# naver/deep-image-retrieval

Hardware: AMD Instinct MI355X
Metric: images/sec descriptor extraction (resnet101-GeM, 1024x1024) (higher is better)
Workload: dtype fp16p

## Files before the change

### deep-image-retrieval_amd/csrc/conv_igemm.hip

```cpp
#include "dir_common.h"
#include "conv_igemm.h"

#include <stdlib.h>
#include <string.h>
#include <algorithm>

namespace dir {

static constexpr uint32_t kOOB = 0x80000000u;

__device__ __forceinline__ void dma16(__amdgpu_buffer_rsrc_t rsrc, char* lds, uint32_t voff, int soff) {
    __builtin_amdgcn_raw_ptr_buffer_load_lds(rsrc, (DIR_LDS void*)lds, 16, voff, soff, 0, 0);
}

__device__ inline uint32_t fast_div(uint32_t n, uint32_t mul, uint32_t shr) {
    return mul ? (__umulhi(n, mul) >> shr) : n;
}

template <class DT, int BM, int BN, int WGM, int WGN, int NST, int BK, bool CIN16, bool SPLITK>
__global__ void __launch_bounds__(64 * WGM * WGN) conv_igemm_kernel(const ConvArgs a) {
    static_assert(NST >= 2 && NST <= 8, "ring depth");
    static_assert((BK == 64 || BK == 32) && (!CIN16 || BK == 64), "K-step");
    constexpr int RB = BK * 2;
    constexpr int CPR = BK / 8;
// ... 552 lines not shown

int conv_pick_dual_variant(const ConvArgs& a, bool any_size) {
    const bool ok = a.x2 && a.R == 1 && a.S == 1 && a.stride == 1 && a.pad == 0 && a.H == a.OH && a.W == a.OW &&
                    a.Cin % 64 == 0 && a.Cin2 % 64 == 0 && a.res == nullptr && a.ksplit <= 1;
    if (!ok) return -1;
    {
        const int v = find_variant("64x256_wregd1x1");
        if (v >= 0 && !env().no_wregd && conv1x1_wregd_admissible(a) &&
            (any_size || (long)ceil_div(a.M, 64) * (a.Cout / 256) >= 1024))
            return v;
    }
    if (a.Cout % 256 != 0 || (!any_size && (long)ceil_div(a.M, 256) * (a.Cout / 256) < 192)) return -1;
    if (env().lc1x1) {
        const int vl = find_variant("256x256_lc1x1");
        if (vl >= 0 && conv1x1_lc_admissible(a)) return vl;
    }
    const int v = find_variant("256x256_persist1x1_x3");
    if (v < 0 || kVariants[v].launch_dual[0] == nullptr) return -1;
    return v;
}

template <class DT>
__global__ void conv_splitk_finalize_kernel(const float* __restrict__ partial, const float* __restrict__ bias,
                                            const uint16_t* res, uint16_t* y,
                                            long total8, int Cout, long MC, int ksplit, int relu, int* ovf_flag) {
    const long i8 = (long)blockIdx.x * blockDim.x + threadIdx.x;
    if (i8 >= total8) return;
    const long o = i8 * 8;
    const int n = (int)(o % Cout);
    float v[8];
    const f32x4_t b0 = *(const DIR_GLOBAL f32x4_t*)(bias + n), b1 = *(const DIR_GLOBAL f32x4_t*)(bias + n + 4);
#pragma unroll
    for (int e = 0; e < 4; ++e) v[e] = b0[e], v[4 + e] = b1[e];
    for (int z = 0; z < ksplit; ++z) {
        const float* p = partial + (size_t)z * MC + o;
        const f32x4_t p0 = *(const DIR_GLOBAL f32x4_t*)p, p1 = *(const DIR_GLOBAL f32x4_t*)(p + 4);
#pragma unroll
        for (int e = 0; e < 4; ++e) v[e] += p0[e], v[4 + e] += p1[e];
    }
    if (res) {
        const u32x4_t rv = gload16(res + o);
#pragma unroll
        for (int e = 0; e < 4; ++e) {
            float lo, hi;
            DT::unpack(rv[e], lo, hi);
            v[2 * e] += lo;
            v[2 * e + 1] += hi;
        }
    }
    if (relu) {
#pragma unroll
        for (int e = 0; e < 8; ++e) v[e] = fmaxf(v[e], 0.f);
    }
    u32x4_t ov;
#pragma unroll
    for (int e = 0; e < 4; ++e) ov[e] = DT::pack(v[2 * e], v[2 * e + 1]);
    gstore16(y + o, ov);
    Ovf<DT> ovf;
    ovf.see(ov);
    ovf.flush(ovf_flag);
}

size_t conv_splitk_bytes(const ConvArgs& a, int ksplit) {
    return ksplit > 1 ? (size_t)ksplit * a.M * a.Cout * sizeof(float) : 0;
}

int conv_splitk_factor(int v, const ConvArgs& a) {
    if (v < 0 || v >= kNumVariants || kVariants[v].launch_sk[0] == nullptr || a.Cin == 16) return 1;
    const ConvVariant& cv = kVariants[v];
    const long tiles = (long)ceil_div(a.M, cv.BM) * (a.Cout / cv.BN);
    const int T = a.Ktot / cv.BK;
    if (tiles > 160 || T < 8) return 1;
    int s = (int)std::min<long>(std::min<long>(8, 512 / tiles), T / 4);
    while (s > 1 && conv_splitk_bytes(a, s) > kSplitKMaxBytes) --s;
    return s < 2 ? 1 : s;
}

int conv_launch(const ConvArgs& a, int dtype, int variant, hipStream_t stream) {
    if (a.Cout % 64 != 0) return fail(DIR_ERR_INVALID, "conv: Cout must be a multiple of 64");
    const bool cin16 = (a.Cin == 16);
    if (cin16) {
        if (a.R != 4 || a.S != 4 || a.stride != 1)
            return fail(DIR_ERR_INVALID, "conv: Cin == 16 is only the 4x4 s1 space-to-depth stem");
    } else if (a.Cin % 64 != 0) {
        return fail(DIR_ERR_INVALID, "conv: Cin must be a multiple of 64 (or 16 for the stem)");
    }
    if (a.R > 4 || a.S > 4) return fail(DIR_ERR_INVALID, "conv: filter larger than 4x4");
    if ((long)a.B * a.H * a.W * a.Cin >= (1L << 30) || (long)a.M * a.Cout >= (1L << 30) ||
        (long)a.Cout * a.Ktot >= (1L << 30))
        return fail(DIR_ERR_INVALID, "conv: tensor exceeds 2^31 bytes; lower the batch");
    if (((uintptr_t)a.x & 15) || ((uintptr_t)a.w & 15) || ((uintptr_t)a.y & 15) ||
        ((uintptr_t)a.res & 15) || ((uintptr_t)a.bias & 15))
        return fail(DIR_ERR_INVALID, "conv: tensors must be 16-byte aligned");
    if (dtype != DIR_BF16 && dtype != DIR_FP16) return fail(DIR_ERR_INVALID, "conv: bad dtype");
    if (a.x2) {
        if (variant < 0) variant = conv_pick_dual_variant(a);
        if (variant < 0 || variant >= kNumVariants || kVariants[variant].launch_dual[0] == nullptr ||
            a.Cout % kVariants[variant].BN != 0 || (kVariants[variant].kind == 9 && !conv1x1_wregd_admissible(a)) || (kVariants[variant].kind == 10 && !conv1x1_lc_admissible(a)) || a.R != 1 || a.S != 1 || a.stride != 1 || a.res || a.ksplit > 1 ||
            a.Cin2 % 64 != 0 || a.Ktot != a.Cin + a.Cin2 || ((uintptr_t)a.x2 & 15) ||
            (long)a.B * a.H2 * a.W2 * a.Cin2 >= (1L << 30))
            return fail(DIR_ERR_INVALID, "conv: no two-source form for this shape / variant");
        hipError_t e = kVariants[variant].launch_dual[dtype](a, stream);
        if (e != hipSuccess)
            return fail(DIR_ERR_HIP, std::string("conv launch ") + kVariants[variant].name + "/dual: " + hipGetErrorString(e));
        return DIR_OK;
    }
    if (variant < 0) variant = conv_pick_variant(a);
    if (!conv_variant_admissible(variant, a))
        return fail(DIR_ERR_INVALID, "conv: variant not admissible for this shape");
    const ConvVariant& cv = kVariants[variant];
    if (a.ksplit > 1) {
        if (cv.launch_sk[0] == nullptr || cin16)
            return fail(DIR_ERR_INVALID, "conv: this variant has no split-K form");
        if (!a.partial || ((uintptr_t)a.partial & 15))
            return fail(DIR_ERR_INVALID, "conv: split-K needs a 16-byte aligned fp32 scratch buffer");
        if (a.ksplit > a.Ktot / cv.BK) return fail(DIR_ERR_INVALID, "conv: more K slices than K-steps");
    }
    hipError_t e = cv.kind == 1   ? conv_patch3x3_launch(a, dtype, stream)
                   : cv.kind == 5 ? conv_patch3x3s_launch(a, dtype, stream)
                   : cv.kind == 6 ? conv_patch3x3w_launch(a, dtype, stream)
                   : cv.kind == 2 ? conv1x1_persist_launch(a, dtype, stream)
                   : cv.kind == 4 ? conv1x1_persist_launch(a, dtype, stream, true)
                   : cv.kind == 3 ? conv1x1_wreg_launch(a, dtype, stream)
#ifdef DIR_EXPERIMENTS
                   : cv.kind == 7 ? conv1x1_ring_launch(a, dtype, stream)
#endif
                   : cv.kind == 8 ? conv_patch64_lc_launch(a, dtype, stream)
                   : cv.kind == 12 ? conv_patch3x3s2_launch(a, dtype, stream)
                   : cv.kind == 10 ? conv1x1_lc_launch(a, dtype, stream)
                   : cv.kind == 11 ? conv_small_launch(a, dtype, cv.stages, stream)
                   : a.ksplit > 1 ? cv.launch_sk[dtype](a, stream)
                                  : (cin16 ? cv.launch16 : cv.launch)[dtype](a, stream);
    if (e != hipSuccess)
        return fail(DIR_ERR_HIP, std::string("conv launch ") + cv.name + ": " + hipGetErrorString(e));
    if (a.ksplit > 1) {
        const long MC = (long)a.M * a.Cout, total8 = MC / 8;
        const dim3 grid((unsigned)((total8 + 255) / 256));
        if (dtype == DIR_BF16)
            hipLaunchKernelGGL(conv_splitk_finalize_kernel<BF16>, grid, dim3(256), 0, stream, a.partial, a.bias,
                               a.res, a.y, total8, a.Cout, MC, a.ksplit, a.relu, a.ovf);
        else
            hipLaunchKernelGGL(conv_splitk_finalize_kernel<FP16>, grid, dim3(256), 0, stream, a.partial, a.bias,
                               a.res, a.y, total8, a.Cout, MC, a.ksplit, a.relu, a.ovf);
        e = hipGetLastError();
        if (e != hipSuccess) return fail(DIR_ERR_HIP, std::string("conv split-K finalize: ") + hipGetErrorString(e));
    }
    return DIR_OK;
}

template <class DT>
__global__ void conv_naive_kernel(const ConvArgs a) {
    const long idx = (long)blockIdx.x * blockDim.x + threadIdx.x;
    if (idx >= (long)a.M * a.Cout) return;
    const int n = (int)(idx % a.Cout);
    const int m = (int)(idx / a.Cout);
    const int OHW = a.OH * a.OW;
    const int b = m / OHW, rem = m - b * OHW, oh = rem / a.OW, ow = rem - oh * a.OW;
    float acc = 0.f;
    for (int r = 0; r < a.R; ++r) {
        const int ih = oh * a.stride - a.pad + r;
        if ((unsigned)ih >= (unsigned)a.H) continue;
        for (int s = 0; s < a.S; ++s) {
            const int iw = ow * a.stride - a.pad + s;
            if ((unsigned)iw >= (unsigned)a.W) continue;
            const uint16_t* xp = a.x + ((size_t)(b * a.H + ih) * a.W + iw) * a.Cin;
            const uint16_t* wp = a.w + (size_t)n * a.Ktot + (r * a.S + s) * a.Cin;
            for (int c = 0; c < a.Cin; ++c) acc = fmaf(DT::to_f32(xp[c]), DT::to_f32(wp[c]), acc);
// ... 24 lines not shown
```

### deep-image-retrieval_amd/csrc/conv_patchw.hip

```cpp
#include "dir_common.h"
#include "conv_igemm.h"

#ifndef DIR_PATCHW_ABL
#define DIR_PATCHW_ABL 0
#endif

namespace dir {

static constexpr uint32_t kOOBw = 0x80000000u;

__device__ __forceinline__ void dma16w(__amdgpu_buffer_rsrc_t rsrc, char* lds, uint32_t voff, int soff) {
    __builtin_amdgcn_raw_ptr_buffer_load_lds(rsrc, (DIR_LDS void*)lds, 16, voff, soff, 0, 0);
}

template <class DT>
__global__ void __launch_bounds__(512) conv_patch3x3w_kernel(const ConvArgs a) {
    constexpr int TH = 16, TW = 32, PH = TH + 2, PW = TW + 2, PP = PH * PW;
    constexpr int NTH = 512, BN = 128;
    constexpr int NPL = (PP * 4 + NTH - 1) / NTH;
    constexpr int PLANE_BYTES = NPL * NTH * 16;
    constexpr int TN = 4, TMR = 2;
    constexpr int WSTAGE = 3 * BN * 64, NBW = WSTAGE / (NTH * 16);
    constexpr int NBW_X = (DIR_PATCHW_ABL & 16) ? 2 : 0;
    constexpr int NPL_X = (DIR_PATCHW_ABL & 32) ? 7 : 0;
    constexpr int NSTW = 3;
    constexpr int WOFF = 2 * PLANE_BYTES;
    constexpr int EROW = TN * 128 + 16;
    typedef typename DT::frag_t frag_t;
    static_assert(WOFF + NSTW * WSTAGE <= 160 * 1024 && NBW * NTH * 16 == WSTAGE, "LDS map");

    extern __shared__ __attribute__((aligned(16))) char smem[];

    const int tid = threadIdx.x;
    const int lane = tid & 63;
    const int wave = __builtin_amdgcn_readfirstlane(tid >> 6);
    const int lrow = lane & 31, lhi = lane >> 5;

    const int NQ = a.Cin / 32;
    const int NS = NQ * 3;
    const int tiles_n = a.Cout / BN;
    const int tiles_x = (a.OW + TW - 1) / TW;
    const int tiles_y = (a.OH + TH - 1) / TH;
    int wg = xcd_remap(blockIdx.x, gridDim.x);
    const int tile_n = wg % tiles_n;
    wg /= tiles_n;
    const int tx = wg % tiles_x;
    wg /= tiles_x;
    const int ty = wg % tiles_y;
    const int b = wg / tiles_y;
    const int oy0 = ty * TH, ox0 = tx * TW;

    const __amdgpu_buffer_rsrc_t rsrc_x = __builtin_amdgcn_make_buffer_rsrc((void*)a.x, 0, a.x_bytes, 0x00020000);
    const __amdgpu_buffer_rsrc_t rsrc_w = __builtin_amdgcn_make_buffer_rsrc((void*)a.w, 0, a.w_bytes, 0x00020000);

    uint32_t pvoff[NPL];
#pragma unroll
    for (int i = 0; i < NPL; ++i) {
        const int P = i * NTH + tid;
        const int p = P >> 2, pos = P & 3;
        const int py = p / PW, px = p - py * PW;
        const int iy = oy0 - 1 + py, ix = ox0 - 1 + px;
        const bool ok = p < PP && (unsigned)iy < (unsigned)a.H && (unsigned)ix < (unsigned)a.W;
        pvoff[i] = ok ? (uint32_t)((((b * a.H + iy) * a.W + ix) * a.Cin + ((pos ^ ((p >> 2) & 3)) << 3)) * 2) : kOOBw;
    }
    auto issue_plane = [&](int q) {
        if (DIR_PATCHW_ABL & 64) return;
        char* dst = smem + (q & 1) * PLANE_BYTES;
#pragma unroll
        for (int i = 0; i < NPL; ++i) dma16w(rsrc_x, dst + (i * NTH + wave * 64) * 16, pvoff[i], q * 64);
#pragma unroll
        for (int rep = 0; rep < NPL_X; ++rep)
#pragma unroll
            for (int i = 0; i < NPL; ++i) dma16w(rsrc_x, dst + (i * NTH + wave * 64) * 16, pvoff[i], q * 64);
    };
    uint32_t wvoff[NBW];
#pragma unroll
    for (int i = 0; i < NBW; ++i) {
        const int L = i * NTH + tid;
        const int s = L >> 9, n = (L & 511) >> 2, pos = L & 3;
        wvoff[i] = (uint32_t)((((tile_n * BN + n) * 9 + s) * a.Cin + ((pos ^ ((n >> 2) & 3)) << 3)) * 2);
    }
    auto issue_w = [&](int sigma, int slot) {
        if (DIR_PATCHW_ABL & 64) return;
        const int q = sigma / 3, r = sigma - q * 3;
        char* dst = smem + WOFF + slot * WSTAGE;
#pragma unroll
        for (int i = 0; i < NBW; ++i) dma16w(rsrc_w, dst + (i * NTH + wave * 64) * 16, wvoff[i], (r * 3 * a.Cin + q * 32) * 2);
#pragma unroll
        for (int i = 0; i < NBW_X; ++i)
            dma16w(rsrc_w, dst + (i * NTH + wave * 64) * 16, wvoff[i], (((r + 1) % 3) * 3 * a.Cin + q * 32) * 2);
    };

    f32x16_t acc[TN][TMR];
#pragma unroll
    for (int i = 0; i < TN; ++i)
#pragma unroll
        for (int g = 0; g < 4; ++g) {
            const f32x4_t b4 = *(const DIR_GLOBAL f32x4_t*)(a.bias + tile_n * BN + i * 32 + 8 * g + 4 * lhi);
#pragma unroll
            for (int j = 0; j < TMR; ++j)
#pragma unroll
                for (int e = 0; e < 4; ++e) acc[i][j][4 * g + e] = b4[e];
        }

    int woffk[2];
#pragma unroll
    for (int kk = 0; kk < 2; ++kk) woffk[kk] = lrow * 64 + (((2 * kk + lhi) ^ ((lrow >> 2) & 3)) << 4);

    issue_plane(0);
    issue_w(0, 0);
    issue_w(1, 1);
    int q = 0, r = 0;
    int slot_c = 0;
    bool plane_before = false;
    for (int sigma = 0; sigma < NS; ++sigma) {
        if (((DIR_PATCHW_ABL & 4) && sigma == 0) || (DIR_PATCHW_ABL & 64)) {
        } else if (sigma + 1 >= NS) {
            asm volatile("s_waitcnt vmcnt(0)" ::: "memory");
        } else if (plane_before) {
            asm volatile("s_waitcnt vmcnt(%0)" ::"i"(NPL * (1 + NPL_X) + NBW + NBW_X) : "memory");
        } else {
            asm volatile("s_waitcnt vmcnt(%0)" ::"i"(NBW + NBW_X) : "memory");
        }
        ring_barrier();
        plane_before = false;
        if (r == 0 && q + 1 < NQ) {
            issue_plane(q + 1);
            plane_before = true;
        }
        if (sigma + 2 < NS) {
            int slot_n = slot_c + 2;
            if (slot_n >= NSTW) slot_n -= NSTW;
            issue_w(sigma + 2, slot_n);
        }
        const char* plane = smem + (q & 1) * PLANE_BYTES;
        const char* wst = smem + WOFF + slot_c * WSTAGE;
#pragma unroll
        for (int s = 0; s < ((DIR_PATCHW_ABL & 128) ? 0 : 3); ++s) {
            frag_t xf[TMR][2], wf[2][TN];
#pragma unroll
            for (int j = 0; j < TMR; ++j) {
                const int p = (wave * TMR + j + r) * PW + s + lrow;
                const int swz = (p >> 2) & 3;
#pragma unroll
                for (int kk = 0; kk < 2; ++kk) xf[j][kk] = *(const frag_t*)(plane + p * 64 + (((2 * kk + lhi) ^ swz) << 4));
            }
#pragma unroll
            for (int kk = 0; kk < 2; ++kk)
#pragma unroll
                for (int i = 0; i < TN; ++i) wf[kk][i] = *(const frag_t*)(wst + s * (BN * 64) + i * 2048 + woffk[kk]);
#pragma unroll
            for (int kk = 0; kk < 2; ++kk)
#pragma unroll
                for (int i = 0; i < TN; ++i)
#pragma unroll
                    for (int j = 0; j < TMR; ++j) {
                        if ((DIR_PATCHW_ABL & 8) && !(s == 0 || (s == 1 && kk == 0 && i < 3))) continue;
                        acc[i][j] = DT::mfma32(wf[kk][i], xf[j][kk], acc[i][j]);
                    }
        }
        asm volatile("s_waitcnt lgkmcnt(0)" ::: "memory");
        if (++slot_c == NSTW) slot_c = 0;
        if (++r == 3) {
            r = 0;
            ++q;
        }
    }
    __syncthreads();
    Ovf<DT> ovf;
    if (DIR_PATCHW_ABL & 2) {
        float sum = 0.f;
#pragma unroll
        for (int i = 0; i < TN; ++i)
#pragma unroll
            for (int j = 0; j < TMR; ++j)
#pragma unroll
                for (int e = 0; e < 16; ++e) sum += acc[i][j][e];
        if (sum == 1.2345678e30f) a.y[0] = 1;
        return;
    }

    char* ebase = smem + wave * (32 * EROW);
    constexpr int LPR = TN * 4, RPP = 64 / LPR, NPASS = 32 / RPP;
    const int ecol = (lane % LPR) * 8;
    const int erow = lane / LPR;
    const int ncol = tile_n * BN + ecol;
#pragma unroll
    for (int j = 0; j < TMR; ++j) {
#pragma unroll
        for (int i = 0; i < TN; ++i)
#pragma unroll
            for (int g = 0; g < 4; ++g) {
                f32x4_t v = {acc[i][j][4 * g + 0], acc[i][j][4 * g + 1], acc[i][j][4 * g + 2], acc[i][j][4 * g + 3]};
                *(f32x4_t*)(ebase + lrow * EROW + (i * 32 + 8 * g + 4 * lhi) * 4) = v;
            }
        __builtin_amdgcn_fence(__ATOMIC_RELEASE, "wavefront");
        __builtin_amdgcn_wave_barrier();
        __builtin_amdgcn_fence(__ATOMIC_ACQUIRE, "wavefront");
        const int oy = oy0 + wave * TMR + j;
#pragma unroll
        for (int pass = 0; pass < NPASS; ++pass) {
            const int mrow = pass * RPP + erow;
            const f32x4_t f0 = *(const f32x4_t*)(ebase + mrow * EROW + ecol * 4);
            const f32x4_t f1 = *(const f32x4_t*)(ebase + mrow * EROW + ecol * 4 + 16);
            const int ox = ox0 + mrow;
            if (oy < a.OH && ox < a.OW) {
                float v[8] = {f0[0], f0[1], f0[2], f0[3], f1[0], f1[1], f1[2], f1[3]};
                const size_t o = ((size_t)(b * a.OH + oy) * a.OW + ox) * a.Cout + ncol;
                if (a.res) {
                    const u32x4_t rv = gload16(a.res + o);
#pragma unroll
                    for (int e = 0; e < 4; ++e) {
                        float lo, hi;
                        DT::unpack(rv[e], lo, hi);
                        v[2 * e] += lo;
                        v[2 * e + 1] += hi;
                    }
                }
                if (a.relu) {
#pragma unroll
                    for (int e = 0; e < 8; ++e) v[e] = fmaxf(v[e], 0.f);
                }
                u32x4_t ov;
#pragma unroll
                for (int e = 0; e < 4; ++e) ov[e] = DT::pack(v[2 * e], v[2 * e + 1]);
                if (!(DIR_PATCHW_ABL & 1) || ov[0] == 0x12345678u) gstore16(a.y + o, ov);
                ovf.see(ov);
            }
        }
        __builtin_amdgcn_fence(__ATOMIC_RELEASE, "wavefront");
        __builtin_amdgcn_wave_barrier();
        __builtin_amdgcn_fence(__ATOMIC_ACQUIRE, "wavefront");
    }
    ovf.flush(a.ovf);
}

template <class DT>
__global__ void __launch_bounds__(768) conv_patch3x3w_lc_kernel(const ConvArgs a) {
    constexpr int TH = 16, TW = 32, PH = TH + 2, PW = TW + 2, PP = PH * PW;
    constexpr int NLD = 256, BN = 128;
    constexpr int NPL = (PP * 4 + NLD - 1) / NLD;
    constexpr int PLANE_BYTES = NPL * NLD * 16;
    constexpr int TN = 4, TMR = 2;
    constexpr int WSTAGE = 3 * BN * 64, NBW = WSTAGE / (NLD * 16);
    constexpr int NSTW = 3;
    constexpr int WOFF = 2 * PLANE_BYTES;
    constexpr int EROW = TN * 128 + 16;
    typedef typename DT::frag_t frag_t;
    static_assert(WOFF + NSTW * WSTAGE <= 160 * 1024 && NBW * NLD * 16 == WSTAGE, "LDS map");

    extern __shared__ __attribute__((aligned(16))) char smem[];

    const int tid = threadIdx.x;
    const int lane = tid & 63;
    const int wave = __builtin_amdgcn_readfirstlane(tid >> 6);
    const int lrow = lane & 31, lhi = lane >> 5;

    const int NQ = a.Cin / 32;
    const int NS = NQ * 3;
    const int tiles_n = a.Cout / BN;
    const int tiles_x = (a.OW + TW - 1) / TW;
    const int tiles_y = (a.OH + TH - 1) / TH;
    int wg = xcd_remap(blockIdx.x, gridDim.x);
    const int tile_n = wg % tiles_n;
    wg /= tiles_n;
    const int tx = wg % tiles_x;
    wg /= tiles_x;
    const int ty = wg % tiles_y;
    const int b = wg / tiles_y;
    const int oy0 = ty * TH, ox0 = tx * TW;

    if (wave >= 8) {
        const int lt = tid - 512;
        const int lw = wave - 8;
        const __amdgpu_buffer_rsrc_t rsrc_x = __builtin_amdgcn_make_buffer_rsrc((void*)a.x, 0, a.x_bytes, 0x00020000);
        uint32_t pvoff[NPL];
#pragma unroll
        for (int i = 0; i < NPL; ++i) {
            const int P = i * NLD + lt;
            const int p = P >> 2, pos = P & 3;
            const int py = p / PW, px = p - py * PW;
            const int iy = oy0 - 1 + py, ix = ox0 - 1 + px;
            const bool ok = p < PP && (unsigned)iy < (unsigned)a.H && (unsigned)ix < (unsigned)a.W;
            pvoff[i] = ok ? (uint32_t)((((b * a.H + iy) * a.W + ix) * a.Cin + ((pos ^ ((p >> 2) & 3)) << 3)) * 2) : kOOBw;
        }
        const bool packed = a.w_pw != nullptr;
        const __amdgpu_buffer_rsrc_t rsrc_wp = __builtin_amdgcn_make_buffer_rsrc((void*)(packed ? a.w_pw : a.w), 0, a.w_bytes, 0x00020000);
        uint32_t wvoff[NBW];
#pragma unroll
        for (int i = 0; i < NBW; ++i) {
            const int L = i * NLD + lt;
            const int s = L >> 9, n = (L & 511) >> 2, pos = L & 3;
            wvoff[i] = packed ? (uint32_t)(L * 16) : (uint32_t)((((tile_n * BN + n) * 9 + s) * a.Cin + ((pos ^ ((n >> 2) & 3)) << 3)) * 2);
        }
        auto issue_plane = [&](int q) {
            char* dst = smem + (q & 1) * PLANE_BYTES;
#pragma unroll
            for (int i = 0; i < NPL; ++i) dma16w(rsrc_x, dst + (i * NLD + lw * 64) * 16, pvoff[i], q * 64);
        };
        auto issue_w = [&](int sigma, int slot) {
            const int q = sigma / 3, r = sigma - q * 3;
            char* dst = smem + WOFF + slot * WSTAGE;
            const int soff = packed ? (tile_n * NS + sigma) * WSTAGE : (r * 3 * a.Cin + q * 32) * 2;
#pragma unroll
            for (int i = 0; i < NBW; ++i) dma16w(rsrc_wp, dst + (i * NLD + lw * 64) * 16, wvoff[i], soff);
        };
        issue_plane(0);
        issue_w(0, 0);
        if (NS > 1) issue_w(1, 1);
        int q = 0, r = 0, slot_c = 0;
        bool plane_before = false;
        for (int sigma = 0; sigma < NS; ++sigma) {
            if (sigma + 1 >= NS) {
                asm volatile("s_waitcnt vmcnt(0)" ::: "memory");
            } else if (plane_before) {
                asm volatile("s_waitcnt vmcnt(%0)" ::"i"(NPL + NBW) : "memory");
            } else {
                asm volatile("s_waitcnt vmcnt(%0)" ::"i"(NBW) : "memory");
            }
            ring_barrier();
            plane_before = false;
            if (r == 0 && q + 1 < NQ) {
                issue_plane(q + 1);
                plane_before = true;
            }
            if (sigma + 2 < NS) {
                int slot_n = slot_c + 2;
                if (slot_n >= NSTW) slot_n -= NSTW;
                issue_w(sigma + 2, slot_n);
            }
            if (++slot_c == NSTW) slot_c = 0;
            if (++r == 3) {
                r = 0;
                ++q;
            }
        }
        ring_barrier();
        return;
    }

    f32x16_t acc[TN][TMR];
#pragma unroll
    for (int i = 0; i < TN; ++i)
#pragma unroll
        for (int g = 0; g < 4; ++g) {
            const f32x4_t b4 = *(const DIR_GLOBAL f32x4_t*)(a.bias + tile_n * BN + i * 32 + 8 * g + 4 * lhi);
#pragma unroll
            for (int j = 0; j < TMR; ++j)
#pragma unroll
                for (int e = 0; e < 4; ++e) acc[i][j][4 * g + e] = b4[e];
        }
    int woffk[2];
#pragma unroll
    for (int kk = 0; kk < 2; ++kk) woffk[kk] = lrow * 64 + (((2 * kk + lhi) ^ ((lrow >> 2) & 3)) << 4);
    asm volatile("s_waitcnt vmcnt(0)" ::: "memory");

    int q = 0, r = 0, slot_c = 0;
    for (int sigma = 0; sigma < NS; ++sigma) {
        ring_barrier();
        const char* plane = smem + (q & 1) * PLANE_BYTES;
        const char* wst = smem + WOFF + slot_c * WSTAGE;
#pragma unroll
        for (int s = 0; s < 3; ++s) {
#pragma unroll
            for (int kk = 0; kk < 2; ++kk) {
                frag_t xf[TMR], wf[TN];
#pragma unroll
                for (int j = 0; j < TMR; ++j) {
                    const int p = (wave * TMR + j + r) * PW + s + lrow;
                    xf[j] = *(const frag_t*)(plane + p * 64 + (((2 * kk + lhi) ^ ((p >> 2) & 3)) << 4));
                }
#pragma unroll
                for (int i = 0; i < TN; ++i) wf[i] = *(const frag_t*)(wst + s * (BN * 64) + i * 2048 + woffk[kk]);
#pragma unroll
                for (int j = 0; j < TMR; ++j)
#pragma unroll
                    for (int i = 0; i < TN; ++i) acc[i][j] = DT::mfma32(wf[i], xf[j], acc[i][j]);
            }
        }
        asm volatile("s_waitcnt lgkmcnt(0)" ::: "memory");
        if (++slot_c == NSTW) slot_c = 0;
        if (++r == 3) {
            r = 0;
            ++q;
        }
    }
    ring_barrier();
    Ovf<DT> ovf;
    char* ebase = smem + wave * (32 * EROW);
    constexpr int LPR = TN * 4, RPP = 64 / LPR, NPASS = 32 / RPP;
    const int ecol = (lane % LPR) * 8;
    const int erow = lane / LPR;
    const int ncol = tile_n * BN + ecol;
#pragma unroll
    for (int j = 0; j < TMR; ++j) {
#pragma unroll
        for (int i = 0; i < TN; ++i)
#pragma unroll
            for (int g = 0; g < 4; ++g) {
                f32x4_t v = {acc[i][j][4 * g + 0], acc[i][j][4 * g + 1], acc[i][j][4 * g + 2], acc[i][j][4 * g + 3]};
                *(f32x4_t*)(ebase + lrow * EROW + (i * 32 + 8 * g + 4 * lhi) * 4) = v;
            }
        __builtin_amdgcn_fence(__ATOMIC_RELEASE, "wavefront");
        __builtin_amdgcn_wave_barrier();
        __builtin_amdgcn_fence(__ATOMIC_ACQUIRE, "wavefront");
        const int oy = oy0 + wave * TMR + j;
#pragma unroll
        for (int pass = 0; pass < NPASS; ++pass) {
            const int mrow = pass * RPP + erow;
            const f32x4_t f0 = *(const f32x4_t*)(ebase + mrow * EROW + ecol * 4);
            const f32x4_t f1 = *(const f32x4_t*)(ebase + mrow * EROW + ecol * 4 + 16);
            const int ox = ox0 + mrow;
            if (oy < a.OH && ox < a.OW) {
                float v[8] = {f0[0], f0[1], f0[2], f0[3], f1[0], f1[1], f1[2], f1[3]};
                const size_t o = ((size_t)(b * a.OH + oy) * a.OW + ox) * a.Cout + ncol;
                if (a.res) {
                    const u32x4_t rv = gload16(a.res + o);
#pragma unroll
                    for (int e = 0; e < 4; ++e) {
                        float lo, hi;
                        DT::unpack(rv[e], lo, hi);
                        v[2 * e] += lo;
                        v[2 * e + 1] += hi;
                    }
                }
                if (a.relu) {
#pragma unroll
                    for (int e = 0; e < 8; ++e) v[e] = fmaxf(v[e], 0.f);
                }
                u32x4_t ov;
#pragma unroll
                for (int e = 0; e < 4; ++e) ov[e] = DT::pack(v[2 * e], v[2 * e + 1]);
                gstore16(a.y + o, ov);
                ovf.see(ov);
            }
        }
        __builtin_amdgcn_fence(__ATOMIC_RELEASE, "wavefront");
        __builtin_amdgcn_wave_barrier();
        __builtin_amdgcn_fence(__ATOMIC_ACQUIRE, "wavefront");
    }
    ovf.flush(a.ovf);
}

bool conv_patch3x3w_admissible(const ConvArgs& a) {
    return a.R == 3 && a.S == 3 && a.stride == 1 && a.pad == 1 && a.H == a.OH && a.W == a.OW && a.Cin % 32 == 0 &&
           a.Cin >= 64 && a.Cout % 128 == 0 && (size_t)a.B * a.H * a.W * a.Cin * 2 < (1ull << 31) &&
           (size_t)a.Cout * a.Ktot * 2 < (1ull << 31);
}

__global__ void __launch_bounds__(256) pack_patchw_kernel(const uint16_t* w, uint16_t* out, int Cout, int Cin) {
    const int NQ = Cin / 32;
    const long pieces = (long)Cout * 9 * Cin / 8;
    for (long i = (long)blockIdx.x * 256 + threadIdx.x; i < pieces; i += (long)gridDim.x * 256) {
        const int L = (int)(i % 1536);
        long t = i / 1536;
        const int r = (int)(t % 3);
        t /= 3;
        const int q = (int)(t % NQ);
        const int tn = (int)(t / NQ);
        const int s = L >> 9, n = (L & 511) >> 2, pos = L & 3;
        const size_t src = ((size_t)((tn * 128 + n) * 9 + r * 3 + s)) * Cin + q * 32 + ((pos ^ ((n >> 2) & 3)) << 3);
        gstore16(out + i * 8, gload16(w + src));
    }
}

hipError_t conv_patch3x3w_pack(const uint16_t* w, uint16_t* out, int Cout, int Cin, hipStream_t stream) {
    const long pieces = (long)Cout * 9 * Cin / 8;
    const int grid = (int)((pieces + 255) / 256 < 1024 ? (pieces + 255) / 256 : 1024);
    hipLaunchKernelGGL(pack_patchw_kernel, dim3(grid), dim3(256), 0, stream, w, out, Cout, Cin);
    return hipGetLastError();
}

template <class DT>
static hipError_t launch_patch_w(const ConvArgs& a, hipStream_t stream) {
    constexpr int LDS = 2 * 5 * 512 * 16 + 3 * 3 * 128 * 64;
    static_assert(LDS <= 160 * 1024 && LDS >= 8 * 32 * (4 * 128 + 16), "LDS map (the staging area aliases it)");
    ConvArgs b = a;
    b.x_bytes = (uint32_t)((size_t)a.B * a.H * a.W * a.Cin * 2);
    b.w_bytes = (uint32_t)((size_t)a.Cout * a.Ktot * 2);
    const long blocks = (long)a.B * ((a.OH + 15) / 16) * ((a.OW + 31) / 32) * (a.Cout / 128);
    if (!env().no_patchw_lc) {
        void* scratch = nullptr;
        if (!b.w_pw && env().patchw_pack) {
            if (hipError_t e = hipMallocAsync(&scratch, b.w_bytes, stream); e != hipSuccess) return e;
            if (hipError_t e = conv_patch3x3w_pack(a.w, (uint16_t*)scratch, a.Cout, a.Cin, stream); e != hipSuccess) {
// ... 29 lines not shown
```

### deep-image-retrieval_amd/csrc/dir_common.h

```cpp
#pragma once
#include <hip/hip_runtime.h>
#include <stdint.h>
#include <string.h>
#include <atomic>
#include <string>

#include "../../include/dir_engine.h"

namespace dir {

typedef __attribute__((ext_vector_type(8))) __bf16 bf16x8_t;
typedef __attribute__((ext_vector_type(8))) _Float16 f16x8_t;
typedef __attribute__((ext_vector_type(16))) float f32x16_t;
typedef __attribute__((ext_vector_type(4))) float f32x4_t;
typedef __attribute__((ext_vector_type(4))) uint32_t u32x4_t;
typedef __attribute__((ext_vector_type(2))) uint32_t u32x2_t;
typedef __attribute__((ext_vector_type(2))) float f32x2_t;
typedef __attribute__((ext_vector_type(2))) __bf16 bf16x2_t;
typedef __attribute__((ext_vector_type(2))) _Float16 f16x2_t;

#define DIR_GLOBAL __attribute__((address_space(1)))
#define DIR_LDS __attribute__((address_space(3)))

void set_error(const std::string& msg);
int fail(int code, const std::string& msg);

#define DIR_HIP_CHECK(expr)                                                                \
    do {                                                                                   \
        hipError_t _e = (expr);                                                            \
        if (_e != hipSuccess)                                                              \
            return ::dir::fail(DIR_ERR_HIP, std::string(#expr) + ": " + hipGetErrorString(_e)); \
    } while (0)

struct Env {
    bool c3c1_off = false, c3c1_force = false;
    bool no_ds_seam = false, no_dual = false;
    bool rev_conv1 = false, rev_conv3 = false;
    bool unfused_stem = false, stem_v1 = false;
    bool no_patchlc = false, no_wreg = false, no_patchw = false, no_x3 = false, no_patchs = false;
    bool patchw_pack = false, no_patchw_pack = false;
    bool small_k2 = false;
    bool no_patchs2 = false;
    bool x3_k2048 = false;
    bool lc1x1 = false;
    bool no_c3c1lc = false;
    bool no_smallmap = false;
    bool no_wregd = false;
    bool no_patchw_lc = false;
    bool no_xcdmap = false;
    bool no_pair_patch = false, pair_acts = false;
    int pair_stages = 1;
    bool sim_v1 = false, sim_exact = false;
    bool experiments = false;
    bool no_inplace = false;
    bool no_stem_u8 = false;
    bool stem_pair_old = false;
    bool stem_u8_prep = false;
    bool stem_u8_wg8 = false;
    int stem_u8_seg = 0;
};
const Env& env();
void reload_env();

__host__ __device__ inline uint16_t f32_to_bf16_bits(float f) {
    uint32_t u;
    memcpy(&u, &f, 4);
    if ((u & 0x7fffffffu) > 0x7f800000u) return (uint16_t)((u >> 16) | 0x40);
    u += 0x7fffu + ((u >> 16) & 1u);
    return (uint16_t)(u >> 16);
}
__host__ __device__ inline float bf16_bits_to_f32(uint16_t h) {
    uint32_t u = ((uint32_t)h) << 16;
    float f;
    memcpy(&f, &u, 4);
    return f;
}
__host__ __device__ inline uint16_t f32_to_f16_bits(float f) {
    _Float16 h = (_Float16)f;
    uint16_t b;
    memcpy(&b, &h, 2);
    return b;
}
__host__ __device__ inline float f16_bits_to_f32(uint16_t b) {
    _Float16 h;
    memcpy(&h, &b, 2);
    return (float)h;
}

struct BF16 {
    typedef bf16x8_t frag_t;
    static constexpr int kDtype = DIR_BF16;
    __host__ __device__ static inline float to_f32(uint16_t b) { return bf16_bits_to_f32(b); }
    __host__ __device__ static inline uint16_t from_f32(float f) { return f32_to_bf16_bits(f); }
    __device__ static inline f32x16_t mfma32(frag_t a, frag_t b, f32x16_t c) {
        return __builtin_amdgcn_mfma_f32_32x32x16_bf16(a, b, c, 0, 0, 0);
    }
    __device__ static inline void unpack(uint32_t w, float& lo, float& hi) {
        lo = __builtin_bit_cast(float, w << 16);
        hi = __builtin_bit_cast(float, w & 0xffff0000u);
    }
    __device__ static inline uint32_t pack(float lo, float hi) {
        const f32x2_t v = {lo, hi};
        return __builtin_bit_cast(uint32_t, __builtin_convertvector(v, bf16x2_t));
    }
};
struct FP16 {
    typedef f16x8_t frag_t;
    static constexpr int kDtype = DIR_FP16;
    __host__ __device__ static inline float to_f32(uint16_t b) { return f16_bits_to_f32(b); }
    __host__ __device__ static inline uint16_t from_f32(float f) { return f32_to_f16_bits(f); }
    __device__ static inline f32x16_t mfma32(frag_t a, frag_t b, f32x16_t c) {
        return __builtin_amdgcn_mfma_f32_32x32x16_f16(a, b, c, 0, 0, 0);
    }
    __device__ static inline void unpack(uint32_t w, float& lo, float& hi) {
        const f32x2_t v = __builtin_convertvector(__builtin_bit_cast(f16x2_t, w), f32x2_t);
        lo = v[0];
        hi = v[1];
    }
    __device__ static inline uint32_t pack(float lo, float hi) {
        const f32x2_t v = {lo, hi};
        return __builtin_bit_cast(uint32_t, __builtin_convertvector(v, f16x2_t));
    }
};

template <class DT>
__device__ inline void unpack2(uint32_t w, float& lo, float& hi) {
    lo = DT::to_f32((uint16_t)(w & 0xffffu));
    hi = DT::to_f32((uint16_t)(w >> 16));
}
template <class DT>
__device__ inline uint32_t pack2(float lo, float hi) {
    return (uint32_t)DT::from_f32(lo) | ((uint32_t)DT::from_f32(hi) << 16);
}

__device__ inline u32x4_t gload16(const void* p) {
    return *(const DIR_GLOBAL u32x4_t*)p;
}
__device__ inline void gstore16(void* p, u32x4_t v) {
    *(DIR_GLOBAL u32x4_t*)p = v;
}

typedef __attribute__((ext_vector_type(2))) uint16_t u16x2_t;
template <class DT>
struct Ovf {
    uint32_t m = 0;
    __device__ inline void see(uint32_t w) {
        if constexpr (DT::kDtype == DIR_FP16) {
            uint32_t t;
            asm("v_and_b32 %1, 0x7fff7fff, %2\n\tv_pk_max_u16 %0, %0, %1" : "+v"(m), "=&v"(t) : "v"(w));
        }
    }
    __device__ inline void see(const u32x4_t& v) {
#pragma unroll
        for (int e = 0; e < 4; ++e) see(v[e]);
    }
    __device__ inline void see(const u32x2_t& v) {
        see(v[0]);
        see(v[1]);
    }
    __device__ inline void flush(int* flag) const {
        if constexpr (DT::kDtype == DIR_FP16) {
            if (flag && ((m + 0x04000400u) & 0x80008000u)) atomicOr(flag, 1);
        }
    }
};

__device__ __forceinline__ void ring_barrier() {
#ifndef DIR_EXP_NO_RING_FENCE
    __builtin_amdgcn_sched_barrier(0);
#endif
    __builtin_amdgcn_s_barrier();
#ifndef DIR_EXP_NO_RING_FENCE
    __builtin_amdgcn_sched_barrier(0);
#endif
}

__device__ inline int xcd_remap(int bid, int nwg) {
    const int q = nwg >> 3, r = nwg & 7, xcd = bid & 7;
    const int start = xcd < r ? xcd * (q + 1) : r * (q + 1) + (xcd - r) * q;
    return start + (bid >> 3);
}

inline int ceil_div(int a, int b) { return (a + b - 1) / b; }

inline int cu_count() {
    static std::atomic<int> cached[64];
    int dev = 0;
    if (hipGetDevice(&dev) != hipSuccess) return 256;
    int n = cached[dev & 63].load(std::memory_order_relaxed);
    if (n > 0) return n;
    hipDeviceProp_t prop;
    n = hipGetDeviceProperties(&prop, dev) == hipSuccess && prop.multiProcessorCount > 0 ? prop.multiProcessorCount : 256;
    cached[dev & 63].store(n, std::memory_order_relaxed);
    return n;
}
// ... 14 lines not shown
```

Before: 2435.

## Rework 3x3 patch conv inner loop to 16x16x32 MFMA with pinned scheduling

```diff
diff --git a/deep-image-retrieval_amd/csrc/conv_igemm.hip b/deep-image-retrieval_amd/csrc/conv_igemm.hip
--- a/deep-image-retrieval_amd/csrc/conv_igemm.hip
+++ b/deep-image-retrieval_amd/csrc/conv_igemm.hip
@@ -658,7 +658,7 @@
     if (cin16) {
         if (a.R != 4 || a.S != 4 || a.stride != 1)
             return fail(DIR_ERR_INVALID, "conv: Cin == 16 is only the 4x4 s1 space-to-depth stem");
-    } else if (a.Cin % 64 != 0) {
+    } else if (a.Cin % 64 != 0 && !(a.Cin % 32 == 0 && !a.x2 && variant >= 0 && variant < kNumVariants && kVariants[variant].kind == 6)) {
         return fail(DIR_ERR_INVALID, "conv: Cin must be a multiple of 64 (or 16 for the stem)");
     }
     if (a.R > 4 || a.S > 4) return fail(DIR_ERR_INVALID, "conv: filter larger than 4x4");
diff --git a/deep-image-retrieval_amd/csrc/conv_patchw.hip b/deep-image-retrieval_amd/csrc/conv_patchw.hip
--- a/deep-image-retrieval_amd/csrc/conv_patchw.hip
+++ b/deep-image-retrieval_amd/csrc/conv_patchw.hip
@@ -13,8 +13,94 @@
     __builtin_amdgcn_raw_ptr_buffer_load_lds(rsrc, (DIR_LDS void*)lds, 16, voff, soff, 0, 0);
 }
 
+#ifndef DIR_PATCHW_ORDER
+#define DIR_PATCHW_ORDER 0
+#endif
+#ifndef DIR_PATCHW_NW
+#define DIR_PATCHW_NW 3
+#endif
+
+template <class DT, int R, int NW = DIR_PATCHW_NW>
+__device__ __forceinline__ void patchw_stage(f32x4_t (&acc)[8][4], const char* smem, uint32_t& xq, uint32_t& u, uint32_t lk,
+                                             uint32_t& wl) {
+    typedef typename DT::frag_t frag_t;
+    constexpr int WSTAGE = 3 * 128 * 64;
+    constexpr bool PIN = !(DIR_PATCHW_ABL & 8);
+    asm volatile("" : "+v"(u), "+v"(wl), "+v"(xq));
+    auto xaddr = [&](int j, int s) -> const char* {
+        const int c = (R + j) * 34 + s;
+        return smem + (xq + ((lk ^ (((u + c) >> 2) & 3)) << 4)) + c * 64;
+    };
+    const char* wp = smem + wl;
+    auto wread = [&](int k) { return *(const frag_t*)(wp + (R * WSTAGE + (k >> 3) * 8192 + (k & 7) * 1024)); };
+    auto live = [](int k) { return !(DIR_PATCHW_ABL & 8) || k < 11; };
+    frag_t xf[4], wf[NW];
+    {
+        const char *a0 = xaddr(0, 0), *a1 = xaddr(1, 0);
+        xf[0] = *(const frag_t*)a0;
+        xf[1] = *(const frag_t*)(a0 + 1024);
+        xf[2] = *(const frag_t*)a1;
+        xf[3] = *(const frag_t*)(a1 + 1024);
+    }
+#pragma unroll
+    for (int k = 0; k < NW; ++k) wf[k] = wread(k);
+    if (PIN) __builtin_amdgcn_sched_group_barrier(0x100, 4 + NW, 0);
+#if DIR_PATCHW_ORDER == 0
+#pragma unroll
+    for (int k = 0; k < 24; ++k) {
+        const int s = k >> 3, i = k & 7;
+        const bool turn = i == 7 && s < 2 && live(k + 1);
+        const char *a0 = smem, *a1 = smem;
+        if (turn) a0 = xaddr(0, s + 1), a1 = xaddr(1, s + 1);
+#pragma unroll
+        for (int x = 0; x < 4; ++x) {
+            if (live(k)) acc[i][x] = DT::mfma16(wf[k % NW], xf[x], acc[i][x]);
+            if (turn) {
+                xf[x] = *(const frag_t*)((x < 2 ? a0 : a1) + (x & 1) * 1024);
+                if (PIN) {
+                    __builtin_amdgcn_sched_group_barrier(0x008, 1, 0);
+                    __builtin_amdgcn_sched_group_barrier(0x100, 1, 0);
+                }
+            }
+        }
+        if (!turn && PIN) __builtin_amdgcn_sched_group_barrier(0x008, 4, 0);
+        if (k + NW < 24 && live(k + NW)) {
+            wf[k % NW] = wread(k + NW);
+            if (PIN) __builtin_amdgcn_sched_group_barrier(0x100, 1, 0);
+        }
+    }
+#else
+#pragma unroll
+    for (int k = 0; k < 24; k += 2) {
+        const int s = k >> 3, i = k & 7;
+        const bool turn = i == 6 && s < 2 && live(k + 2);
+        const char *a0 = smem, *a1 = smem;
+        if (turn) a0 = xaddr(0, s + 1), a1 = xaddr(1, s + 1);
+#pragma unroll
+        for (int x = 0; x < 4; ++x) {
+            if (live(k)) acc[i][x] = DT::mfma16(wf[k % NW], xf[x], acc[i][x]);
+            if (PIN) __builtin_amdgcn_sched_group_barrier(0x008, 1, 0);
+            if (x == 3 && k + 3 < 24 && live(k + 3)) {
+                wf[k % NW] = wread(k + 3);
+                if (PIN) __builtin_amdgcn_sched_group_barrier(0x100, 1, 0);
+            }
+            if (live(k + 1)) acc[i + 1][x] = DT::mfma16(wf[(k + 1) % NW], xf[x], acc[i + 1][x]);
+            if (PIN) __builtin_amdgcn_sched_group_barrier(0x008, 1, 0);
+            if (turn) {
+                xf[x] = *(const frag_t*)((x < 2 ? a0 : a1) + (x & 1) * 1024);
+                if (PIN) __builtin_amdgcn_sched_group_barrier(0x100, 1, 0);
+            }
+        }
+        if (k + 4 < 24 && live(k + 4)) {
+            wf[(k + 1) % NW] = wread(k + 4);
+            if (PIN) __builtin_amdgcn_sched_group_barrier(0x100, 1, 0);
+        }
+    }
+#endif
+}
+
 template <class DT>
-__global__ void __launch_bounds__(512) conv_patch3x3w_kernel(const ConvArgs a) {
+__global__ void __launch_bounds__(512) __attribute__((amdgpu_waves_per_eu(3, 3))) conv_patch3x3w_kernel(const ConvArgs a) {
     constexpr int TH = 16, TW = 32, PH = TH + 2, PW = TW + 2, PP = PH * PW;
     constexpr int NTH = 512, BN = 128;
     constexpr int NPL = (PP * 4 + NTH - 1) / NTH;
@@ -26,7 +112,6 @@
     constexpr int NSTW = 3;
     constexpr int WOFF = 2 * PLANE_BYTES;
     constexpr int EROW = TN * 128 + 16;
-    typedef typename DT::frag_t frag_t;
     static_assert(WOFF + NSTW * WSTAGE <= 160 * 1024 && NBW * NTH * 16 == WSTAGE, "LDS map");
 
     extern __shared__ __attribute__((aligned(16))) char smem[];
@@ -34,7 +119,7 @@
     const int tid = threadIdx.x;
     const int lane = tid & 63;
     const int wave = __builtin_amdgcn_readfirstlane(tid >> 6);
-    const int lrow = lane & 31, lhi = lane >> 5;
+    const int l15 = lane & 15, lk = lane >> 4;
 
     const int NQ = a.Cin / 32;
     const int NS = NQ * 3;
@@ -53,147 +138,111 @@
     const __amdgpu_buffer_rsrc_t rsrc_x = __builtin_amdgcn_make_buffer_rsrc((void*)a.x, 0, a.x_bytes, 0x00020000);
     const __amdgpu_buffer_rsrc_t rsrc_w = __builtin_amdgcn_make_buffer_rsrc((void*)a.w, 0, a.w_bytes, 0x00020000);
 
-    uint32_t pvoff[NPL];
-#pragma unroll
-    for (int i = 0; i < NPL; ++i) {
-        const int P = i * NTH + tid;
-        const int p = P >> 2, pos = P & 3;
-        const int py = p / PW, px = p - py * PW;
-        const int iy = oy0 - 1 + py, ix = ox0 - 1 + px;
-        const bool ok = p < PP && (unsigned)iy < (unsigned)a.H && (unsigned)ix < (unsigned)a.W;
-        pvoff[i] = ok ? (uint32_t)((((b * a.H + iy) * a.W + ix) * a.Cin + ((pos ^ ((p >> 2) & 3)) << 3)) * 2) : kOOBw;
-    }
+    int tid_p = tid;
     auto issue_plane = [&](int q) {
         if (DIR_PATCHW_ABL & 64) return;
+        asm volatile("" : "+v"(tid_p));
         char* dst = smem + (q & 1) * PLANE_BYTES;
 #pragma unroll
-        for (int i = 0; i < NPL; ++i) dma16w(rsrc_x, dst + (i * NTH + wave * 64) * 16, pvoff[i], q * 64);
-#pragma unroll
-        for (int rep = 0; rep < NPL_X; ++rep)
-#pragma unroll
-            for (int i = 0; i < NPL; ++i) dma16w(rsrc_x, dst + (i * NTH + wave * 64) * 16, pvoff[i], q * 64);
+        for (int rep = 0; rep < 1 + NPL_X; ++rep)
+#pragma unroll
+            for (int i = 0; i < NPL; ++i) {
+                const int P = i * NTH + tid_p;
+                const int p = P >> 2, pos = P & 3;
+                const int py = p / PW, px = p - py * PW;
+                const int iy = oy0 - 1 + py, ix = ox0 - 1 + px;
+                const bool ok = p < PP && (unsigned)iy < (unsigned)a.H && (unsigned)ix < (unsigned)a.W;
+                const uint32_t off = (uint32_t)((((b * a.H + iy) * a.W + ix) * a.Cin + ((pos ^ ((p >> 2) & 3)) << 3)) * 2);
+                dma16w(rsrc_x, dst + (i * NTH + wave * 64) * 16, off | (ok ? 0u : kOOBw), q * 64);
+            }
     };
-    uint32_t wvoff[NBW];
-#pragma unroll
-    for (int i = 0; i < NBW; ++i) {
-        const int L = i * NTH + tid;
-        const int s = L >> 9, n = (L & 511) >> 2, pos = L & 3;
-        wvoff[i] = (uint32_t)((((tile_n * BN + n) * 9 + s) * a.Cin + ((pos ^ ((n >> 2) & 3)) << 3)) * 2);
-    }
+    static_assert(NBW == 3 && NTH == 512, "one tap per weight DMA instruction");
+    const uint32_t wvoff = (uint32_t)(((tile_n * BN + (tid >> 2)) * 9 * a.Cin + (((tid & 3) ^ ((tid >> 4) & 3)) << 3)) * 2);
     auto issue_w = [&](int sigma, int slot) {
         if (DIR_PATCHW_ABL & 64) return;
         const int q = sigma / 3, r = sigma - q * 3;
         char* dst = smem + WOFF + slot * WSTAGE;
 #pragma unroll
-        for (int i = 0; i < NBW; ++i) dma16w(rsrc_w, dst + (i * NTH + wave * 64) * 16, wvoff[i], (r * 3 * a.Cin + q * 32) * 2);
+        for (int i = 0; i < NBW; ++i) dma16w(rsrc_w, dst + (i * NTH + wave * 64) * 16, wvoff, ((r * 3 + i) * a.Cin + q * 32) * 2);
 #pragma unroll
         for (int i = 0; i < NBW_X; ++i)
-            dma16w(rsrc_w, dst + (i * NTH + wave * 64) * 16, wvoff[i], (((r + 1) % 3) * 3 * a.Cin + q * 32) * 2);
+            dma16w(rsrc_w, dst + (i * NTH + wave * 64) * 16, wvoff, ((((r + 1) % 3) * 3 + i) * a.Cin + q * 32) * 2);
     };
 
-    f32x16_t acc[TN][TMR];
-#pragma unroll
-    for (int i = 0; i < TN; ++i)
-#pragma unroll
-        for (int g = 0; g < 4; ++g) {
-            const f32x4_t b4 = *(const DIR_GLOBAL f32x4_t*)(a.bias + tile_n * BN + i * 32 + 8 * g + 4 * lhi);
-#pragma unroll
-            for (int j = 0; j < TMR; ++j)
-#pragma unroll
-                for (int e = 0; e < 4; ++e) acc[i][j][4 * g + e] = b4[e];
-        }
-
-    int woffk[2];
-#pragma unroll
-    for (int kk = 0; kk < 2; ++kk) woffk[kk] = lrow * 64 + (((2 * kk + lhi) ^ ((lrow >> 2) & 3)) << 4);
+    f32x4_t acc[8][4];
+#pragma unroll
+    for (int i = 0; i < 8; ++i) {
+        const f32x4_t b4 = *(const DIR_GLOBAL f32x4_t*)(a.bias + tile_n * BN + i * 16 + 4 * lk);
+#pragma unroll
+        for (int x = 0; x < 4; ++x) acc[i][x] = b4;
+    }
+
+    uint32_t u = wave * (TMR * PW) + l15;
+    uint32_t wl = WOFF + l15 * 64 + ((lk ^ ((l15 >> 2) & 3)) << 4);
 
     issue_plane(0);
     issue_w(0, 0);
     issue_w(1, 1);
-    int q = 0, r = 0;
-    int slot_c = 0;
-    bool plane_before = false;
-    for (int sigma = 0; sigma < NS; ++sigma) {
+    auto stage_begin = [&](int q, auto R_, auto LAST_) {
+        constexpr int r = decltype(R_)::value;
+        constexpr bool LAST = decltype(LAST_)::value;
+        const int sigma = q * 3 + r;
         if (((DIR_PATCHW_ABL & 4) && sigma == 0) || (DIR_PATCHW_ABL & 64)) {
-        } else if (sigma + 1 >= NS) {
+        } else if (LAST && r == 2) {
             asm volatile("s_waitcnt vmcnt(0)" ::: "memory");
-        } else if (plane_before) {
+        } else if (r == 1 && !LAST) {
             asm volatile("s_waitcnt vmcnt(%0)" ::"i"(NPL * (1 + NPL_X) + NBW + NBW_X) : "memory");
         } else {
             asm volatile("s_waitcnt vmcnt(%0)" ::"i"(NBW + NBW_X) : "memory");
         }
         ring_barrier();
-        plane_before = false;
-        if (r == 0 && q + 1 < NQ) {
-            issue_plane(q + 1);
-            plane_before = true;
-        }
-        if (sigma + 2 < NS) {
-            int slot_n = slot_c + 2;
-            if (slot_n >= NSTW) slot_n -= NSTW;
-            issue_w(sigma + 2, slot_n);
-        }
-        const char* plane = smem + (q & 1) * PLANE_BYTES;
-        const char* wst = smem + WOFF + slot_c * WSTAGE;
-#pragma unroll
-        for (int s = 0; s < ((DIR_PATCHW_ABL & 128) ? 0 : 3); ++s) {
-            frag_t xf[TMR][2], wf[2][TN];
-#pragma unroll
-            for (int j = 0; j < TMR; ++j) {
-                const int p = (wave * TMR + j + r) * PW + s + lrow;
-                const int swz = (p >> 2) & 3;
-#pragma unroll
-                for (int kk = 0; kk < 2; ++kk) xf[j][kk] = *(const frag_t*)(plane + p * 64 + (((2 * kk + lhi) ^ swz) << 4));
-            }
-#pragma unroll
-            for (int kk = 0; kk < 2; ++kk)
-#pragma unroll
-                for (int i = 0; i < TN; ++i) wf[kk][i] = *(const frag_t*)(wst + s * (BN * 64) + i * 2048 + woffk[kk]);
-#pragma unroll
-            for (int kk = 0; kk < 2; ++kk)
-#pragma unroll
-                for (int i = 0; i < TN; ++i)
-#pragma unroll
-                    for (int j = 0; j < TMR; ++j) {
-                        if ((DIR_PATCHW_ABL & 8) && !(s == 0 || (s == 1 && kk == 0 && i < 3))) continue;
-                        acc[i][j] = DT::mfma32(wf[kk][i], xf[j][kk], acc[i][j]);
-                    }
-        }
+        if (r == 0 && !LAST) issue_plane(q + 1);
+        if (r == 0 || !LAST) issue_w(sigma + 2, (r + 2) % NSTW);
+    };
+    auto plane_stages = [&](int q, auto LAST_) {
+        uint32_t xq = u * 64 + (q & 1) * PLANE_BYTES;
+        stage_begin(q, std::integral_constant<int, 0>(), LAST_);
+        if (!(DIR_PATCHW_ABL & 128)) patchw_stage<DT, 0, 2>(acc, smem, xq, u, lk, wl);
         asm volatile("s_waitcnt lgkmcnt(0)" ::: "memory");
-        if (++slot_c == NSTW) slot_c = 0;
-        if (++r == 3) {
-            r = 0;
-            ++q;
-        }
-    }
-    __syncthreads();
+        stage_begin(q, std::integral_constant<int, 1>(), LAST_);
+        if (!(DIR_PATCHW_ABL & 128)) patchw_stage<DT, 1, 2>(acc, smem, xq, u, lk, wl);
+        asm volatile("s_waitcnt lgkmcnt(0)" ::: "memory");
+        stage_begin(q, std::integral_constant<int, 2>(), LAST_);
+        if (!(DIR_PATCHW_ABL & 128)) patchw_stage<DT, 2, 2>(acc, smem, xq, u, lk, wl);
+        asm volatile("s_waitcnt lgkmcnt(0)" ::: "memory");
+    };
+    for (int q = 0; q + 1 < NQ; ++q) plane_stages(q, std::false_type());
+    int nq_end = NQ;
+    asm volatile("" : "+s"(nq_end));
+    for (int q = NQ - 1; q < nq_end; ++q) plane_stages(q, std::true_type());
+    ring_barrier();
     Ovf<DT> ovf;
     if (DIR_PATCHW_ABL & 2) {
         float sum = 0.f;
 #pragma unroll
-        for (int i = 0; i < TN; ++i)
-#pragma unroll
-            for (int j = 0; j < TMR; ++j)
-#pragma unroll
-                for (int e = 0; e < 16; ++e) sum += acc[i][j][e];
+        for (int i = 0; i < 8; ++i)
+#pragma unroll
+            for (int x = 0; x < 4; ++x)
+#pragma unroll
+                for (int e = 0; e < 4; ++e) sum += acc[i][x][e];
         if (sum == 1.2345678e30f) a.y[0] = 1;
         return;
     }
 
     char* ebase = smem + wave * (32 * EROW);
     constexpr int LPR = TN * 4, RPP = 64 / LPR, NPASS = 32 / RPP;
-    const int ecol = (lane % LPR) * 8;
-    const int erow = lane / LPR;
+    int lane_e = tid_p & 63;
+    asm volatile("" : "+v"(lane_e));
+    const int ecol = (lane_e % LPR) * 8;
+    const int erow = lane_e / LPR;
+    const int l15e = lane_e & 15, lke = lane_e >> 4;
     const int ncol = tile_n * BN + ecol;
 #pragma unroll
     for (int j = 0; j < TMR; ++j) {
 #pragma unroll
-        for (int i = 0; i < TN; ++i)
-#pragma unroll
-            for (int g = 0; g < 4; ++g) {
-                f32x4_t v = {acc[i][j][4 * g + 0], acc[i][j][4 * g + 1], acc[i][j][4 * g + 2], acc[i][j][4 * g + 3]};
-                *(f32x4_t*)(ebase + lrow * EROW + (i * 32 + 8 * g + 4 * lhi) * 4) = v;
-            }
+        for (int i = 0; i < 8; ++i)
+#pragma unroll
+            for (int h = 0; h < 2; ++h) *(f32x4_t*)(ebase + (h * 16 + l15e) * EROW + (i * 16 + 4 * lke) * 4) = acc[i][2 * j + h];
         __builtin_amdgcn_fence(__ATOMIC_RELEASE, "wavefront");
         __builtin_amdgcn_wave_barrier();
         __builtin_amdgcn_fence(__ATOMIC_ACQUIRE, "wavefront");
@@ -246,7 +295,6 @@
     constexpr int NSTW = 3;
     constexpr int WOFF = 2 * PLANE_BYTES;
     constexpr int EROW = TN * 128 + 16;
-    typedef typename DT::frag_t frag_t;
     static_assert(WOFF + NSTW * WSTAGE <= 160 * 1024 && NBW * NLD * 16 == WSTAGE, "LDS map");
 
     extern __shared__ __attribute__((aligned(16))) char smem[];
@@ -254,7 +302,7 @@
     const int tid = threadIdx.x;
     const int lane = tid & 63;
     const int wave = __builtin_amdgcn_readfirstlane(tid >> 6);
-    const int lrow = lane & 31, lhi = lane >> 5;
+    const int l15 = lane & 15, lk = lane >> 4;
 
     const int NQ = a.Cin / 32;
     const int NS = NQ * 3;
@@ -339,68 +387,44 @@
         return;
     }
 
-    f32x16_t acc[TN][TMR];
-#pragma unroll
-    for (int i = 0; i < TN; ++i)
-#pragma unroll
-        for (int g = 0; g < 4; ++g) {
-            const f32x4_t b4 = *(const DIR_GLOBAL f32x4_t*)(a.bias + tile_n * BN + i * 32 + 8 * g + 4 * lhi);
-#pragma unroll
-            for (int j = 0; j < TMR; ++j)
-#pragma unroll
-                for (int e = 0; e < 4; ++e) acc[i][j][4 * g + e] = b4[e];
-        }
-    int woffk[2];
-#pragma unroll
-    for (int kk = 0; kk < 2; ++kk) woffk[kk] = lrow * 64 + (((2 * kk + lhi) ^ ((lrow >> 2) & 3)) << 4);
+    f32x4_t acc[8][4];
+#pragma unroll
+    for (int i = 0; i < 8; ++i) {
+        const f32x4_t b4 = *(const DIR_GLOBAL f32x4_t*)(a.bias + tile_n * BN + i * 16 + 4 * lk);
+#pragma unroll
+        for (int x = 0; x < 4; ++x) acc[i][x] = b4;
+    }
+    uint32_t u = wave * (TMR * PW) + l15;
+    uint32_t wl = WOFF + l15 * 64 + ((lk ^ ((l15 >> 2) & 3)) << 4);
     asm volatile("s_waitcnt vmcnt(0)" ::: "memory");
 
-    int q = 0, r = 0, slot_c = 0;
-    for (int sigma = 0; sigma < NS; ++sigma) {
+    for (int q = 0; q < NQ; ++q) {
+        uint32_t xq = u * 64 + (q & 1) * PLANE_BYTES;
         ring_barrier();
-        const char* plane = smem + (q & 1) * PLANE_BYTES;
-        const char* wst = smem + WOFF + slot_c * WSTAGE;
-#pragma unroll
-        for (int s = 0; s < 3; ++s) {
-#pragma unroll
-            for (int kk = 0; kk < 2; ++kk) {
-                frag_t xf[TMR], wf[TN];
-#pragma unroll
-                for (int j = 0; j < TMR; ++j) {
-                    const int p = (wave * TMR + j + r) * PW + s + lrow;
-                    xf[j] = *(const frag_t*)(plane + p * 64 + (((2 * kk + lhi) ^ ((p >> 2) & 3)) << 4));
-                }
-#pragma unroll
-                for (int i = 0; i < TN; ++i) wf[i] = *(const frag_t*)(wst + s * (BN * 64) + i * 2048 + woffk[kk]);
-#pragma unroll
-                for (int j = 0; j < TMR; ++j)
-#pragma unroll
-                    for (int i = 0; i < TN; ++i) acc[i][j] = DT::mfma32(wf[i], xf[j], acc[i][j]);
-            }
-        }
+        patchw_stage<DT, 0>(acc, smem, xq, u, lk, wl);
         asm volatile("s_waitcnt lgkmcnt(0)" ::: "memory");
-        if (++slot_c == NSTW) slot_c = 0;
-        if (++r == 3) {
-            r = 0;
-            ++q;
-        }
+        ring_barrier();
+        patchw_stage<DT, 1>(acc, smem, xq, u, lk, wl);
+        asm volatile("s_waitcnt lgkmcnt(0)" ::: "memory");
+        ring_barrier();
+        patchw_stage<DT, 2>(acc, smem, xq, u, lk, wl);
+        asm volatile("s_waitcnt lgkmcnt(0)" ::: "memory");
     }
     ring_barrier();
     Ovf<DT> ovf;
     char* ebase = smem + wave * (32 * EROW);
     constexpr int LPR = TN * 4, RPP = 64 / LPR, NPASS = 32 / RPP;
-    const int ecol = (lane % LPR) * 8;
-    const int erow = lane / LPR;
+    int lane_e = l15 + 16 * lk;
+    asm volatile("" : "+v"(lane_e));
+    const int ecol = (lane_e % LPR) * 8;
+    const int erow = lane_e / LPR;
     const int ncol = tile_n * BN + ecol;
 #pragma unroll
     for (int j = 0; j < TMR; ++j) {
 #pragma unroll
-        for (int i = 0; i < TN; ++i)
-#pragma unroll
-            for (int g = 0; g < 4; ++g) {
-                f32x4_t v = {acc[i][j][4 * g + 0], acc[i][j][4 * g + 1], acc[i][j][4 * g + 2], acc[i][j][4 * g + 3]};
-                *(f32x4_t*)(ebase + lrow * EROW + (i * 32 + 8 * g + 4 * lhi) * 4) = v;
-            }
+        for (int i = 0; i < 8; ++i)
+#pragma unroll
+            for (int h = 0; h < 2; ++h) *(f32x4_t*)(ebase + (h * 16 + l15) * EROW + (i * 16 + 4 * lk) * 4) = acc[i][2 * j + h];
         __builtin_amdgcn_fence(__ATOMIC_RELEASE, "wavefront");
         __builtin_amdgcn_wave_barrier();
         __builtin_amdgcn_fence(__ATOMIC_ACQUIRE, "wavefront");
diff --git a/deep-image-retrieval_amd/csrc/dir_common.h b/deep-image-retrieval_amd/csrc/dir_common.h
--- a/deep-image-retrieval_amd/csrc/dir_common.h
+++ b/deep-image-retrieval_amd/csrc/dir_common.h
@@ -95,6 +95,9 @@
     __device__ static inline f32x16_t mfma32(frag_t a, frag_t b, f32x16_t c) {
         return __builtin_amdgcn_mfma_f32_32x32x16_bf16(a, b, c, 0, 0, 0);
     }
+    __device__ static inline f32x4_t mfma16(frag_t a, frag_t b, f32x4_t c) {
+        return __builtin_amdgcn_mfma_f32_16x16x32_bf16(a, b, c, 0, 0, 0);
+    }
     __device__ static inline void unpack(uint32_t w, float& lo, float& hi) {
         lo = __builtin_bit_cast(float, w << 16);
         hi = __builtin_bit_cast(float, w & 0xffff0000u);
@@ -111,6 +114,9 @@
     __host__ __device__ static inline uint16_t from_f32(float f) { return f32_to_f16_bits(f); }
     __device__ static inline f32x16_t mfma32(frag_t a, frag_t b, f32x16_t c) {
         return __builtin_amdgcn_mfma_f32_32x32x16_f16(a, b, c, 0, 0, 0);
+    }
+    __device__ static inline f32x4_t mfma16(frag_t a, frag_t b, f32x4_t c) {
+        return __builtin_amdgcn_mfma_f32_16x16x32_f16(a, b, c, 0, 0, 0);
     }
     __device__ static inline void unpack(uint32_t w, float& lo, float& hi) {
         const f32x2_t v = __builtin_convertvector(__builtin_bit_cast(f16x2_t, w), f32x2_t);
```

Result: no change. 2438 (median of 6 runs) (+0.2%).
